# pl0q1n/RustyHGI

Measured on AMD Instinct MI355X. Metric: Mpixels/s encode+decode, 4K grayscale level=4 Medium, higher is better.
Workload: dtype u8

## Files before the change

rustyhgi_amd/csrc/hgi_capi.hip:

```cpp
#include <hip/hip_runtime.h>
#include <stdarg.h>
#include <stdio.h>
#include <stdlib.h>
#include <string.h>
#include <cstring>
#include <thread>
#include <vector>

#include "hgi_framelist.h"
#include "hgi_host.h"
#include "hgi_pitched.h"

using namespace hgi;
using namespace hgi::host;

namespace {
thread_local char g_err[512] = "";
}

namespace hgi {
namespace host {

hgi_status fail(hgi_status st, const char *fmt, ...)
{
    va_list ap;
    va_start(ap, fmt);
    vsnprintf(g_err, sizeof(g_err), fmt, ap);
    va_end(ap);
    return st;
}

}
}

namespace {

#ifndef HGI_ENC_L1_TILE_ROWS
#define HGI_ENC_L1_TILE_ROWS 16
#endif
#ifndef HGI_TILE16_MAX
#define HGI_TILE16_MAX 600
#endif
constexpr uint32_t kConeMinLevels = 6;

}

namespace hgi {
namespace host {

hgi_status ws_ensure(hgi_ctx *c, size_t bytes)
{
    if (bytes <= c->ws_bytes) return HGI_OK;
    HIP_TRY(hipStreamSynchronize(c->stream));
    if (c->ws) HIP_TRY(hipFree(c->ws));
    c->ws = nullptr;
    c->ws_bytes = 0;
    HIP_TRY(hipMalloc(reinterpret_cast<void **>(&c->ws), bytes));
    c->ws_bytes = bytes;
    return HGI_OK;
}

uint8_t *ws_take(hgi_ctx *c, size_t bytes)
{
    size_t off = align_up(c->ws_used, 256);
    if (off + bytes > c->ws_bytes) return nullptr;
    c->ws_used = off + bytes;
    return c->ws + off;
}

struct SubGeom {
    uint32_t sw, sh;
    uint64_t stride;
};

SubGeom sub_geom(uint32_t w, uint32_t h, uint32_t k)
{
    SubGeom g;
    g.sw = (uint32_t)((((uint64_t)w - 1) >> k) + 1);
    g.sh = (uint32_t)((((uint64_t)h - 1) >> k) + 1);
    g.stride = align_up((size_t)g.sw * g.sh, 256);
    return g;
}

struct Split {
    uint32_t k, up, shift;
};

Split split_pyramid(uint32_t levels)
{
    if (levels < kConeMinLevels) return {levels, 0u, 0u};
    if (levels <= 8u) return {4u, levels - 4u, 0u};
    return {4u, 4u, 8u};
}

size_t plane_bytes(const SubGeom &g, size_t batch) { return align_up(batch * g.stride, 256) + 256; }

size_t ws_need_decode(uint32_t w, uint32_t h, uint32_t levels, size_t batch)
{
    const Split sp = split_pyramid(levels);
    if (!sp.shift) return 0;
    const SubGeom g = sub_geom(w, h, sp.shift);
    return 2 * plane_bytes(g, batch) + ws_need_decode(g.sw, g.sh, levels - sp.shift, batch);
}

size_t ws_need_encode(uint32_t w, uint32_t h, uint32_t levels, size_t batch)
{
    const Split sp = split_pyramid(levels);
    if (!sp.shift) return 0;
    const SubGeom g = sub_geom(w, h, sp.shift);
    return 3 * plane_bytes(g, batch) + ws_need_encode(g.sw, g.sh, levels - sp.shift, batch) + ws_need_decode(g.sw, g.sh, levels - sp.shift, batch);
}

size_t ws_need(const hgi_ctx *c, uint32_t w, uint32_t h, uint32_t levels, size_t batch, size_t stride)
{
    if (levels == 0) return 0;
    if (c->path == HGI_PATH_LEVELWISE) return align_up(batch * stride, 256) + 256;
    const size_t e = ws_need_encode(w, h, levels, batch), d = ws_need_decode(w, h, levels, batch);
    return e > d ? e : d;
}

uint32_t use_tile_rows(uint32_t w, uint32_t h, uint32_t k, size_t batch, bool encode, bool plain)
{
    const int forced = HGI_KNOB(HGI_TILE_H, 0);
    const uint64_t tiny_max = (uint64_t)HGI_KNOB(HGI_TILE16_MAX, HGI_TILE16_MAX);
    if (k > (uint32_t)kFusedMaxLevelsSmall) return 64;
    const bool fits16 = k <= (uint32_t)kFusedMaxLevelsTiny;
    if (forced == 16 && fits16) return 16;
    if (forced == 32 || (forced == 16 && !fits16)) return 32;
    if (forced == 64) return 64;
    const uint64_t tx = (w + kTileW - 1) / kTileW;
    const uint64_t tiles64 = tx * ((h + 63) / 64) * batch, tiles32 = tx * ((h + 31) / 32) * batch;
    if (encode && fits16 && tiles32 <= tiny_max) return 16;
    if (tiles64 < 1536) return 32;
    if (encode && plain && k == 1 && w <= 8192) return HGI_ENC_L1_TILE_ROWS;
    const uint64_t interior64 = (uint64_t)(w / kTileW) * (h / 64) * batch * kTileW * 64;
    if (encode && plain && w <= 8192 && interior64 < ((uint64_t)kEncodeEighthsFromGiB << 30)) return 32;
    return 64;
}

bool use_lattice_kernel(const SubGeom &g, size_t batch)
{
    return !HGI_SWITCH(HGI_NO_LATTICE_KERNEL) && lattice_pyramid_fits(g.sw, g.sh, batch);
}

hipError_t launch_encode_fused(const uint8_t *img, uint8_t *grid, const Frames &f, uint32_t k, int interp,
                               const Lut256 &lut, bool ident, const Seeds *seeds, hipStream_t s, uint32_t row_limit = 0)
{
    const uint32_t rows = row_limit && row_limit < f.height ? row_limit : f.height;
    switch (use_tile_rows(f.width, rows, k, f.batch, true, seeds == nullptr)) {
    case 16: return launch_encode_fused_16(img, grid, f, k, interp, lut, ident, seeds, s, row_limit);
    case 32: return launch_encode_fused_32(img, grid, f, k, interp, lut, ident, seeds, s, row_limit);
    default: return launch_encode_fused_64(img, grid, f, k, interp, lut, ident, seeds, s, row_limit);
    }
}

hipError_t launch_decode_fused(const uint8_t *grid, uint8_t *img, const Frames &f, uint32_t k, int interp,
                               const Seeds *seeds, hipStream_t s, uint32_t row_limit = 0, int resident_tiles = -1)
{
    const uint32_t rows = row_limit && row_limit < f.height ? row_limit : f.height;
    switch (use_tile_rows(f.width, rows, k, f.batch, false, seeds == nullptr)) {
    case 16: return launch_decode_fused_16(grid, img, f, k, interp, seeds, s, row_limit, resident_tiles);
    case 32: return launch_decode_fused_32(grid, img, f, k, interp, seeds, s, row_limit, resident_tiles);
    default: return launch_decode_fused_64(grid, img, f, k, interp, seeds, s, row_limit, resident_tiles);
    }
}

Lut256 pack_lut(const uint8_t lut[256])
{
    Lut256 l;
    memcpy(l.w, lut, 256);
    return l;
}

bool is_identity(const uint8_t lut[256])
{
    for (int i = 0; i < 256; ++i)
        if (lut[i] != i) return false;
    return true;
}

hgi_status encode_impl(hgi_ctx *c, const uint8_t *img, uint32_t w, uint32_t h, uint32_t levels, int interp,
                       const uint8_t lut[256], uint8_t *grid, size_t batch, size_t stride)
{
    Frames f = {w, h, (uint64_t)stride, (uint32_t)batch};
    if (levels == 0) {
        for (size_t b = 0; b < batch; ++b)
            HIP_TRY(launch_copy(img + b * stride, grid + b * stride, (size_t)w * h, c->stream));
        return HGI_OK;
    }
    Lut256 l = pack_lut(lut);
    if (c->path == HGI_PATH_LEVELWISE) {
        uint8_t *rec = ws_take(c, batch * stride);
        if (!rec) return fail(HGI_ENOMEM, "scratch exhausted (level-wise reconstruction plane)");
        HIP_TRY(launch_copy(img, rec, (batch - 1) * stride + (size_t)w * h, c->stream));
        HIP_TRY(launch_seed(img, grid, f, levels, c->stream));
        for (uint32_t level = 0; level < levels; ++level)
            HIP_TRY(launch_encode_level(rec, grid, f, levels - level - 1, interp, l, c->stream));
        return HGI_OK;
    }
    const Split sp = split_pyramid(levels);
    if (sp.shift) {
        const SubGeom g = sub_geom(w, h, sp.shift);
        uint8_t *sub_img = ws_take(c, batch * g.stride);
        uint8_t *sub_grid = ws_take(c, batch * g.stride);
        uint8_t *sub_rec = ws_take(c, batch * g.stride);
        if (!sub_img || !sub_grid || !sub_rec) return fail(HGI_ENOMEM, "scratch exhausted (lattice planes)");
        if (use_lattice_kernel(g, batch)) {
            HIP_TRY(launch_lattice_pyramid(img, f, sp.shift, levels - sp.shift, interp, l, is_identity(lut), true, sub_grid, sub_rec,
                                           g.sw, g.sh, g.stride, c->stream));
        } else {
            HIP_TRY(launch_gather_lattice(img, f, sp.shift, sub_img, g.sw, g.sh, g.stride, c->stream));
            HGI_TRY(encode_impl(c, sub_img, g.sw, g.sh, levels - sp.shift, interp, lut, sub_grid, batch, g.stride));
            HGI_TRY(decode_impl(c, sub_grid, g.sw, g.sh, levels - sp.shift, interp, sub_rec, batch, g.stride));
// ... 1124 lines not shown
```

rustyhgi_amd/csrc/hgi_fused_impl.h:

```cpp
#include "hgi_dev.h"
#include "hgi_fastdiv.h"
#include "hgi_knobs.h"
#include "hgi_tilewalk.h"

namespace hgi {
namespace {

using namespace dev;

#ifndef HGI_TILE_H
#define HGI_TILE_H 64
#endif
#define HGI_LOG2(v) ((v) == 32 ? 5 : (v) == 16 ? 4 : (v) == 8 ? 3 : (v) == 4 ? 2 : 1)
#define HGI_CAT2(a, b) a##_##b
#define HGI_CAT(a, b) HGI_CAT2(a, b)
#define HGI_TILED(name) HGI_CAT(name, HGI_TILE_H)
#define HGI_LANE ((int)threadIdx.x)
constexpr int TW = kTileW;
constexpr int TH = HGI_TILE_H;
constexpr int MAXK = TH == 64 ? kFusedMaxLevels : TH == 32 ? kFusedMaxLevelsSmall : kFusedMaxLevelsTiny;
constexpr int NL = kThreads;
constexpr int CH = TW / 16;
constexpr int LCH = 3;
constexpr int HR = 6;
#ifndef HGI_S_PAD
#define HGI_S_PAD 16
#endif
#ifndef HGI_S2_PAD
#define HGI_S2_PAD 8
#endif
constexpr int S = TW + HGI_S_PAD;
constexpr int HP = 40;
constexpr int HCOL = -(HR * HP);
constexpr int S2 = TW / 2 + HGI_S2_PAD;
constexpr int HP2 = 40;
constexpr int RCOL = -(HR * HP2);

__host__ __device__ constexpr int buf_bytes(int nh) { return HR * HP + (TH / 2 + nh) * S; }
__host__ __device__ constexpr int rbuf_bytes(int nh) { return HR * HP2 + (TH / 2 + nh) * S2; }

static_assert(NL == 64 && CH == (1 << LCH) && (TH & (TH - 1)) == 0 && (TH == 64 || TH == 32 || TH == 16) && (1 << MAXK) <= TH, "tile geometry");
static_assert(S % 16 == 0 && (HR * HP) % 16 == 0 && S2 % 8 == 0 && (HR * HP2) % 16 == 0 && HP >= TH / 2 + HR &&
                  HP2 >= TH / 2 + HR && buf_bytes(1) % 16 == 0 && rbuf_bytes(1) % 8 == 0,
              "LDS pitches keep vector alignment");
#ifdef HGI_FUSED_DECODE
static_assert(TH != 64 || 24 * buf_bytes(4) <= 160 * 1024, "LDS budget: 24 decode waves per CU at k = 4");
#endif
#ifdef HGI_FUSED_ENCODE
static_assert(TH != 64 || 18 * (buf_bytes(4) + rbuf_bytes(4) + 256) <= 160 * 1024, "LDS budget: 18 encode waves per CU at k = 4");
#endif

#ifndef HGI_LOAD_AUX
#define HGI_LOAD_AUX 0
#endif
#ifndef HGI_ODD_LOAD_AUX
#define HGI_ODD_LOAD_AUX 2
#endif
#ifndef HGI_STORE_AUX
#define HGI_STORE_AUX 2
#endif
#ifndef HGI_ODD_LATE
#define HGI_ODD_LATE 1
#endif
#ifndef HGI_DEC_CONE_FIRST
#define HGI_DEC_CONE_FIRST 0
#endif
#ifndef HGI_DEC_SHALLOW_WAVES
#define HGI_DEC_SHALLOW_WAVES 20
#endif
#ifndef HGI_DEC_DEEP_WAVES
#define HGI_DEC_DEEP_WAVES 16
#endif
#ifndef HGI_DEC_STREAM_WAVES
#define HGI_DEC_STREAM_WAVES 10
#endif
#ifndef HGI_DEC_STREAM_WAVES_WIDE
#define HGI_DEC_STREAM_WAVES_WIDE 12
#endif
#ifndef HGI_DEC_STREAM_WAVES_L1
#define HGI_DEC_STREAM_WAVES_L1 8
#endif
#ifndef HGI_XCD_MODE
#define HGI_XCD_MODE -1
#endif
#ifndef HGI_XCD_EIGHTHS_FROM_GIB
#define HGI_XCD_EIGHTHS_FROM_GIB kEncodeEighthsFromGiB
#endif
#ifndef HGI_DEC_REVERSE_DEFAULT
#define HGI_DEC_REVERSE_DEFAULT 0
#endif
#ifndef HGI_TILE_BAND
#define HGI_TILE_BAND 8
#endif
#ifndef HGI_HALO_FIRST
#define HGI_HALO_FIRST 0
#endif
#ifndef HGI_HALO_ALL_ROWS
#define HGI_HALO_ALL_ROWS 0
#endif
#ifdef HGI_ANALYZE_K
#define HGI_MARK(name) asm volatile("; HGI_MARK " name)
#else
#define HGI_MARK(name)
#endif
typedef u32 v4u __attribute__((ext_vector_type(4)));
typedef u32 v2u __attribute__((ext_vector_type(2)));
typedef u32 v3u __attribute__((ext_vector_type(3)));

#define HGI_ADDB(dst, K, src, J)                                                                    \
    asm("v_add_u16_sdwa %0, %0, %1 dst_sel:BYTE_" #K " dst_unused:UNUSED_PRESERVE src0_sel:BYTE_" #K \
        " src1_sel:BYTE_" #J                                                                        \
        : "+v"(dst)                                                                                 \
        : "v"(src))

typedef unsigned long long lanemask;
typedef __attribute__((address_space(3))) const u8 lds_cu8;
__device__ __forceinline__ u32 lut_at(u32 d) { return *(lds_cu8 *)(size_t)d; }
#define Q_SUB(d, a, K, p, J)                                                                                   \
    asm("v_sub_u16_sdwa %0, %1, %2 dst_sel:BYTE_0 dst_unused:UNUSED_PAD src0_sel:BYTE_" #K " src1_sel:BYTE_" #J \
        : "=v"(d) : "v"(a), "v"(p))
#define Q_LT(m, a, K, p, J) \
    asm("v_cmp_lt_u16_sdwa %0, %1, %2 src0_sel:BYTE_" #K " src1_sel:BYTE_" #J : "=s"(m) : "v"(a), "v"(p))
#define Q_GT(m, q, np, J) \
    asm("v_cmp_gt_u16_sdwa %0, %1, %2 src0_sel:BYTE_0 src1_sel:BYTE_" #J : "=s"(m) : "v"(q), "v"(np))
#define Q_SEL(out, K, mb, mc, q, d)                                                                    \
    asm("s_xor_b64 vcc, %1, %2\n\tv_cndmask_b32_sdwa %0, %3, %4, vcc dst_sel:BYTE_" #K                 \
        " dst_unused:UNUSED_PRESERVE src0_sel:BYTE_0 src1_sel:BYTE_0"                                  \
        : "+v"(out) : "s"(mb), "s"(mc), "v"(q), "v"(d) : "vcc", "scc")
#define Q_PIX4(slut, P, NP, O0, K0, J0, O1, K1, J1, O2, K2, J2, O3, K3, J3)                              \
    do {                                                                                               \
        u32 d0_, d1_, d2_, d3_;                                                                        \
        lanemask b0_, b1_, b2_, b3_, c0_, c1_, c2_, c3_;                                               \
        Q_SUB(d0_, O0, K0, P, J0); Q_SUB(d1_, O1, K1, P, J1); Q_SUB(d2_, O2, K2, P, J2); Q_SUB(d3_, O3, K3, P, J3); \
        u32 q0_ = lut_at(d0_), q1_ = lut_at(d1_), q2_ = lut_at(d2_), q3_ = lut_at(d3_);                \
        Q_LT(b0_, O0, K0, P, J0); Q_LT(b1_, O1, K1, P, J1); Q_LT(b2_, O2, K2, P, J2); Q_LT(b3_, O3, K3, P, J3); \
        Q_GT(c0_, q0_, NP, J0); Q_GT(c1_, q1_, NP, J1); Q_GT(c2_, q2_, NP, J2); Q_GT(c3_, q3_, NP, J3); \
        Q_SEL(O0, K0, b0_, c0_, q0_, d0_); Q_SEL(O1, K1, b1_, c1_, q1_, d1_);                          \
        Q_SEL(O2, K2, b2_, c2_, q2_, d2_); Q_SEL(O3, K3, b3_, c3_, q3_, d3_);                          \
    } while (0)
// ... 856 lines not shown
}

__device__ __forceinline__ u8 *uniform_ptr(const u8 *p)
{
    const u64 a = reinterpret_cast<u64>(p);
    const u32 lo = __builtin_amdgcn_readfirstlane((u32)a), hi = __builtin_amdgcn_readfirstlane((u32)(a >> 32));
    return reinterpret_cast<u8 *>(((u64)hi << 32) | lo);
}

__device__ __forceinline__ Buf make_buf(const u8 *fr, u8 *out, u32 W, u32 H, Tile tl, u32 tail)
{
    Buf b;
    const u32 bytes = W * H;
    b.rs = __builtin_amdgcn_make_buffer_rsrc(uniform_ptr(fr), 0, bytes + tail, 0x00020000);
    b.rd = __builtin_amdgcn_make_buffer_rsrc(uniform_ptr(out), 0, bytes, 0x00020000);
    b.W = W;
    b.base = __builtin_amdgcn_readfirstlane(tl.Y0 * W + tl.X0);
    return b;
}

__device__ __forceinline__ Tile fast_tile(u32 t, const TileGrid &g)
{
    t = __builtin_amdgcn_readfirstlane(walk_position(t, g));
    const WalkTile w = walk_fast_tile(t, g);
    Tile tl;
    tl.frame = w.frame;
    tl.X0 = w.tx * TW;
    tl.Y0 = w.ty * TH;
    return tl;
}

__device__ __forceinline__ Tile edge_tile(u32 e, const TileGrid &g)
{
    const WalkTile w = walk_edge_tile(e, g);
    Tile tl;
    tl.frame = w.frame;
    tl.X0 = w.tx * TW;
    tl.Y0 = w.ty * TH;
    return tl;
}

struct TileCtx {
    Tile tl;
    Buf b;
};

#ifndef HGI_ARGS_EARLY
#define HGI_ARGS_EARLY 1
#endif
__device__ __forceinline__ void args_early(const u8 *src, const u8 *dst, const Frames &f, const TileGrid &g, u32 aligned, u32 k)
{
#if HGI_ARGS_EARLY
    asm volatile("" ::"s"(k), "s"(g.full_x), "s"(g.full_y), "s"(g.tiles_x), "s"(g.tiles_y));
    asm volatile("" ::"s"(src), "s"(dst), "s"(f.width), "s"(f.height), "s"(f.frame_stride), "s"(aligned), "s"(g.nedge), "s"(g.nf), "s"(g.xmode),
                 "s"(g.rr_own), "s"(g.rr_tail0), "s"(g.P), "s"(g.fd_P.m), "s"(g.fd_P.s1), "s"(g.fd_P.s2), "s"(g.reverse), "s"(g.tpf), "s"(g.fd_tpf.m),
                 "s"(g.fd_tpf.s1), "s"(g.fd_tpf.s2), "s"(g.nfull), "s"(g.rem_rows), "s"(g.band), "s"(g.ex), "s"(g.fd_band.m), "s"(g.fd_band.s1),
                 "s"(g.fd_band.s2), "s"(g.fd_rem.m), "s"(g.fd_rem.s1), "s"(g.fd_rem.s2));
#endif
}

__device__ __forceinline__ TileCtx fast_ctx(u32 t, const u8 *src, u8 *dst, const Frames &f, const TileGrid &g, u32 tail)
{
    TileCtx c;
    c.tl = fast_tile(t, g);
    c.b = make_buf(src + (size_t)c.tl.frame * f.frame_stride, dst + (size_t)c.tl.frame * f.frame_stride, f.width,
                   f.height, c.tl, tail);
    return c;
}

struct SeedRegs {
    u32 rec, q;
    int bx, by;
    bool on;
};

template <bool WANT_Q>
__device__ __forceinline__ SeedRegs seed_issue(const Seeds &sd, Tile tl, u32 k)
{
    const int ext = k >= 2 ? 2 : 1;
    const int nbx = (TW >> k) + ext, nby = (TH >> k) + ext;
    const int i = HGI_LANE;
    SeedRegs r;
    r.by = i / nbx;
    r.bx = i - r.by * nbx;
    r.on = i < nbx * nby;
    r.rec = r.q = 0;
    const u32 sx = (tl.X0 >> k) + r.bx, sy = (tl.Y0 >> k) + r.by;
    if (r.on && sx < sd.sw && sy < sd.sh) {
        const size_t at = (size_t)tl.frame * sd.stride + (size_t)sy * sd.sw + sx;
        r.rec = sd.rec[at];
        if (WANT_Q) r.q = sd.q[at];
    }
    return r;
}

__device__ __forceinline__ void dec_seed_commit(u8 *buf, const SeedRegs &r, u32 k)
{
    if (r.on) buf[laddr(r.bx << k, r.by << k)] = (u8)r.rec;
    LDS_ORDER();
}

constexpr int kConeMaxUp = 4;
__host__ __device__ constexpr int cone_n(int tile_px, int t)
{
    const int c = tile_px >> 4;
    int n = c + 2;
    for (int i = 0; i < t; ++i) n = (c % (2 << i) == 0 ? (n - 1) / 2 : n / 2) + 2;
// ... 386 lines not shown
        if (tl.X0 + TW <= W && !(H & 1u))
            enc_tile_edge<INTERP, IDENT, 1>(buf, rbuf, slut, cur, st.o, k, W, H);
        else
            enc_tile_edge<INTERP, IDENT, 2>(buf, rbuf, slut, cur, st.o, k, W, H);
        return;
    }
    if (!IDENT) reinterpret_cast<u32 *>(slut)[HGI_LANE] = lut.w[HGI_LANE];
    stage_tile_generic(buf, fr, W, H, tl, nh, (aligned & 1u) != 0);
    LDS_ORDER();
    lattice_from_buf(buf, rbuf, nh);
    LDS_ORDER();
    if (SEEDED == 2) seeds = cone_finish<INTERP, true, IDENT>(cone, buf, rbuf, sd.up, slut);
    enc_seed_commit<SEEDED>(buf, rbuf, seeds, k);
    for (int s = 1 << (k - 1); s >= 2; s >>= 1) {
        enc_cells<INTERP, IDENT, true>(buf, rbuf, slut, s, tl, W, H);
        enc_halo_pass<INTERP, IDENT>(buf, rbuf, slut, s, tl, W, H);
        LDS_ORDER();
    }
    enc_fine_generic<INTERP, IDENT>(buf, rbuf, slut, fr, out, tl, W, H, (aligned & 1u) != 0);
}

inline bool ptr16(const void *p) { return (reinterpret_cast<uintptr_t>(p) & 15u) == 0; }

struct FusedGeom {
    TileGrid g;
    u32 aligned;
    bool ok;
};

FusedGeom fused_geom(const void *a, const void *b, const Frames &f, u32 row_limit)
{
    FusedGeom r;
    TileGrid &g = r.g;
    g.tiles_x = (f.width + TW - 1) / TW;
    g.tiles_y = (f.height + TH - 1) / TH;
    if (row_limit && row_limit / TH < g.tiles_y) g.tiles_y = row_limit / TH;
    const bool aligned = f.width % 16 == 0 && f.frame_stride % 16 == 0 && ptr16(a) && ptr16(b);
    const bool fits32 = ((u64)f.height + 2 * TH + 64) * f.width + 1024 < (1ull << 32);
    const bool force_checked = HGI_SWITCH(HGI_FORCE_CHECKED);
    const uintptr_t end = reinterpret_cast<uintptr_t>(a) + (uintptr_t)(f.batch - 1) * f.frame_stride + (uintptr_t)f.width * f.height;
    const bool dword_rows = f.width % 4 == 0;
    const bool tail_ok = ((end - 1) >> 12) == ((end + 2) >> 12) && (f.batch == 1 || f.frame_stride >= (u64)f.width * f.height);
    const bool fast = fits32 && (dword_rows || tail_ok) && !force_checked;
    g.full_x = fast ? f.width / TW : 0;
    g.full_y = fast ? f.height / TH : 0;
    if (g.full_y > g.tiles_y) g.full_y = g.tiles_y;
    if (g.full_x == 0 || g.full_y == 0) g.full_x = g.full_y = 0;
    const u64 all = (u64)g.tiles_x * g.tiles_y * f.batch, nfast = (u64)g.full_x * g.full_y * f.batch;
    r.ok = all > 0 && all + 8 < (1ull << 31);
    g.nfast = (u32)nfast;
    g.nedge = (u32)(all - nfast);
    g.reverse = 0;
    g.band = HGI_TILE_BAND;
    g.xmode = 0;
    r.aligned = (aligned ? 1u : 0u) | (fast ? 2u : 0u) | (fast && !dword_rows ? 4u : 0u);
#ifdef HGI_TIMELINE
    g.timeline = g_timeline;
#endif
    return r;
}

inline u32 band_rows(const Frames &f, bool encode)
{
    const int forced = encode ? HGI_KNOB(HGI_ENC_BAND, 0) : HGI_KNOB(HGI_DEC_BAND, 0);
    if (forced > 0) return (u32)forced;
    const u64 cap = encode ? (4u << 20) : (2u << 20);
    u32 rows = HGI_TILE_BAND;
    while (rows > 1 && (u64)rows * TH * f.width > cap) rows >>= 1;
    return rows;
}


inline size_t lds_for_waves(size_t lds, int waves)
{
    if (waves <= 0) return lds;
    const size_t cap = ((size_t)160 * 1024 / (size_t)waves) & ~(size_t)255;
    return cap > lds ? cap : lds;
}

inline u32 xcd_mode(const TileGrid &g, bool encode)
{
    const int forced = HGI_KNOB(HGI_XCD_MODE, HGI_XCD_MODE);
    if (forced >= 0) return (u32)forced;
    return encode && (u64)g.nfast * TW * TH >= ((u64)HGI_XCD_EIGHTHS_FROM_GIB << 30) ? 0u : 1u;
}

}

#ifndef HGI_FUSED_NO_LAUNCHERS
#ifdef HGI_FUSED_DECODE
hipError_t HGI_TILED(launch_decode_fused)(const uint8_t *grid, uint8_t *img, const Frames &f, uint32_t k, int interp,
                                          const Seeds *seeds, hipStream_t s, uint32_t row_limit, int resident_tiles)
{
    FusedGeom r = fused_geom(grid, img, f, row_limit);
    if (!r.ok || k < 1 || k > (u32)MAXK) return hipErrorInvalidValue;
    r.g.reverse = HGI_KNOB(HGI_DEC_REVERSE, HGI_DEC_REVERSE_DEFAULT) ? 1u : 0u;
    r.g.band = band_rows(f, false);
    r.g.xmode = xcd_mode(r.g, false);
    finish_grid(r.g);
    const TileGrid &g = r.g;
    if (seeds && k < (uint32_t)kSeededMinLevels) return hipErrorInvalidValue;
    Seeds sd = seeds ? *seeds : Seeds{nullptr, nullptr, 0, 0, 0, 0};
    const bool cone = seeds && seeds->up != 0;
    if (cone && (k != 4 || sd.up > (u32)kConeMaxUp)) return hipErrorInvalidValue;
    if (seeds && !cone && !seeds->rec) return hipErrorInvalidValue;
    const dim3 b(NL);
    const int nh = k >= 2 ? (int)k : 1;
    const int dec_waves_forced = HGI_KNOB(HGI_DEC_WAVES, -1);
    const u64 tiles = (u64)g.nfast + g.nedge;
    int dec_waves = 0;
    if (resident_tiles >= 0)
        dec_waves = resident_tiles;
    else if (dec_waves_forced >= 0)
        dec_waves = dec_waves_forced;
    else if (tiles < 8192)
        dec_waves = 0;
    else if (!seeds)
        dec_waves = f.width > 4096 || k > 4 ? HGI_DEC_STREAM_WAVES_WIDE : k == 1 ? HGI_DEC_STREAM_WAVES_L1 : HGI_DEC_STREAM_WAVES;
    else
        dec_waves = tiles >= 65536 ? HGI_DEC_DEEP_WAVES : HGI_DEC_SHALLOW_WAVES;
    const size_t lds = lds_for_waves((size_t)buf_bytes(nh), dec_waves);
    const dim3 blocks(((g.nedge + 7u) & ~7u) + g.nfast);
#define HGI_DEC(I, SE) hipLaunchKernelGGL((k_dec_tiles<I, SE, TH>), blocks, b, lds, s, grid, img, f, k, sd, g, r.aligned)
#define HGI_DEC_I(I)                                                     \
    do {                                                                 \
        if (!seeds) HGI_DEC(I, 0);                                       \
        else if (cone) HGI_DEC(I, 2);                                    \
        else if constexpr (TH == 64) HGI_DEC(I, 1);                      \
        else return hipErrorInvalidValue;                                \
    } while (0)
    if (interp == kInterpCrossed) HGI_DEC_I(kInterpCrossed); else HGI_DEC_I(kInterpLeftTop);
#undef HGI_DEC_I
#undef HGI_DEC
    return hipGetLastError();
}

#endif

#ifdef HGI_FUSED_ENCODE
namespace {
hipError_t static_lds_is_empty(const void *kernel)
{
    hipFuncAttributes a;
    const hipError_t e = hipFuncGetAttributes(&a, kernel);
    if (e != hipSuccess) return e;
    return a.sharedSizeBytes == 0 ? hipSuccess : hipErrorInvalidDeviceFunction;
}
}

hipError_t HGI_TILED(launch_encode_fused)(const uint8_t *img, uint8_t *grid, const Frames &f, uint32_t k, int interp,
                                          const Lut256 &lut, bool ident, const Seeds *seeds, hipStream_t s, uint32_t row_limit)
{
    FusedGeom r = fused_geom(img, grid, f, row_limit);
    if (!r.ok || k < 1 || k > (u32)MAXK) return hipErrorInvalidValue;
    r.g.band = band_rows(f, true);
    r.g.xmode = xcd_mode(r.g, true);
    finish_grid(r.g);
    const TileGrid &g = r.g;
    if (seeds && k < (uint32_t)kSeededMinLevels) return hipErrorInvalidValue;
    Seeds sd = seeds ? *seeds : Seeds{nullptr, nullptr, 0, 0, 0, 0};
    const bool cone = seeds && seeds->up != 0;
    if (cone && (k != 4 || sd.up > (u32)kConeMaxUp)) return hipErrorInvalidValue;
    if (seeds && (!seeds->rec != !seeds->q || (!cone && !seeds->rec))) return hipErrorInvalidValue;
    const dim3 b(NL);
    const int nh = k >= 2 ? (int)k : 1;
    const int enc_waves = HGI_KNOB(HGI_ENC_WAVES, 0);
    const size_t lds = lds_for_waves((size_t)buf_bytes(nh) + ((rbuf_bytes(nh) + 15) & ~15) + 256, enc_waves);
    const dim3 blocks(((g.nedge + 7u) & ~7u) + g.nfast);
#define HGI_ENC(I, ID, SE)                                                                                        \
    do {                                                                                                          \
        static const hipError_t lds0 = static_lds_is_empty(reinterpret_cast<const void *>(&k_enc_tiles<I, ID, SE, TH>)); \
        if (lds0 != hipSuccess) return lds0;                                                                      \
        hipLaunchKernelGGL((k_enc_tiles<I, ID, SE, TH>), blocks, b, lds, s, img, grid, f, k, lut, sd, g, r.aligned); \
    } while (0)
#define HGI_ENC_ID(I, ID)                                                     \
    do {                                                                      \
        if (cone) HGI_ENC(I, ID, 2);                                          \
        else if (!seeds) HGI_ENC(I, ID, 0);                                   \
        else if constexpr (TH == 64) HGI_ENC(I, ID, 1);                       \
        else return hipErrorInvalidValue;                                     \
    } while (0)
#define HGI_ENC_I(I)                                                          \
    do {                                                                      \
        if (ident) HGI_ENC_ID(I, true); else HGI_ENC_ID(I, false);            \
    } while (0)
    if (interp == kInterpCrossed) HGI_ENC_I(kInterpCrossed); else HGI_ENC_I(kInterpLeftTop);
#undef HGI_ENC_I
#undef HGI_ENC_ID
#undef HGI_ENC
    return hipGetLastError();
}

#endif
#endif

}
```

rustyhgi_amd/csrc/hgi_kernels.h:

```cpp
#pragma once
#include <hip/hip_runtime.h>
#include <stddef.h>
#include <stdint.h>

#include "hgi_huffman_host.h"

namespace hgi {

constexpr int kInterpLeftTop = 0;
constexpr int kInterpCrossed = 1;

constexpr int kTileW = 128;
constexpr int kFusedMaxLevels = 6;
constexpr int kFusedMaxLevelsSmall = 5;
constexpr int kFusedMaxLevelsTiny = 4;
constexpr int kSeededMinLevels = 4;
constexpr int kThreads = 64;
constexpr int kEncodeEighthsFromGiB = 4;

struct Lut256 {
    uint32_t w[64];
};

struct Frames {
    uint32_t width, height;
    uint64_t frame_stride;
    uint32_t batch;
};

struct Seeds {
    const uint8_t *rec;
    const uint8_t *q;
    uint32_t sw, sh;
    uint64_t stride;
    uint32_t up;
};

#ifdef HGI_TIMELINE
extern uint64_t *g_timeline;
#endif

hipError_t launch_seed(const uint8_t *src, uint8_t *dst, const Frames &f, uint32_t levels,
                       hipStream_t s);
hipError_t launch_decode_level(const uint8_t *grid, uint8_t *img, const Frames &f, uint32_t log2sub,
                               int interp, hipStream_t s);
hipError_t launch_encode_level(uint8_t *rec, uint8_t *grid, const Frames &f, uint32_t log2sub,
                               int interp, const Lut256 &lut, hipStream_t s);

#define HGI_DECLARE_FUSED(TH)                                                                                      \
    hipError_t launch_decode_fused_##TH(const uint8_t *grid, uint8_t *img, const Frames &f, uint32_t k, int interp, \
                                        const Seeds *seeds, hipStream_t s, uint32_t row_limit, int resident_tiles); \
    hipError_t launch_encode_fused_##TH(const uint8_t *img, uint8_t *grid, const Frames &f, uint32_t k, int interp, \
                                        const Lut256 &lut, bool lut_is_identity, const Seeds *seeds, hipStream_t s, \
                                        uint32_t row_limit);
HGI_DECLARE_FUSED(64)
HGI_DECLARE_FUSED(32)
HGI_DECLARE_FUSED(16)
#undef HGI_DECLARE_FUSED

struct RegionRect {
    uint32_t x0, y0, width, height;
    uint64_t out_pitch, out_frame_stride;
};
hipError_t launch_decode_region(const uint8_t *grid, uint8_t *out, const Frames &f, const RegionRect &r, uint32_t k, int interp,
                                const Seeds *seeds, hipStream_t s);

struct ScaledView {
    uint32_t width, height, shift;
    uint64_t row_pitch, frame_bytes, frame_stride;
    uint32_t batch;
    uint64_t out_pitch, out_frame_stride;
// ... 40 lines not shown
```

rustyhgi_amd/csrc/hgi_planes.hip:

```cpp
#include <hip/hip_runtime.h>
#include <stdarg.h>
#include <stdio.h>
#include <stdlib.h>
#include <array>
#include <mutex>
#include <utility>
#include <vector>

#include "hgi_host.h"
#include "hgi_lineup.h"

using namespace hgi;
using namespace hgi::host;
using hgi::lineup::arrange;

namespace {

hgi_status probe_pair_ms(hgi_ctx *c, const uint8_t *prev, uint8_t *cand, size_t bytes, float *ms)
{
    const uint32_t w = 4096;
    size_t rows = bytes / w;
    if (rows > (2u << 20) / 4) rows = (2u << 20) / 4;
    rows &= ~(size_t)63;
    const uint32_t h = (uint32_t)rows;
    constexpr int kWarm = 2, kTimed = 4;
    struct Occupancy {
        hgi_ctx *c;
        explicit Occupancy(hgi_ctx *ctx) : c(ctx) { c->probe_resident_tiles = 0; }
        ~Occupancy() { c->probe_resident_tiles = -1; }
    } occupancy(c);
    for (int i = 0; i < kWarm + kTimed; ++i) {
        if (i == kWarm) HIP_TRY(hipEventRecord(c->ev_probe[0], c->stream));
        c->ws_used = 0;
        HGI_TRY(decode_impl(c, prev, w, h, 4, HGI_INTERP_LEFTTOP, cand, 1, (size_t)w * h));
    }
    HIP_TRY(hipEventRecord(c->ev_probe[1], c->stream));
    HIP_TRY(hipEventSynchronize(c->ev_probe[1]));
    HIP_TRY(hipEventElapsedTime(ms, c->ev_probe[0], c->ev_probe[1]));
    *ms /= kTimed;
    return HGI_OK;
}

constexpr size_t kGiB = (size_t)1 << 30;
constexpr float kFastRatio = 0.972f, kUnsureLo = 0.962f, kUnsureHi = 0.985f;
constexpr int kMaxCandidates = 10;
constexpr size_t kComposeAbove = kGiB;
constexpr size_t kChunk = kGiB;

struct Yardstick {
    void *ref = nullptr;
    uint8_t *lo = nullptr, *hi = nullptr;
    size_t span = 0;

    hgi_status make(size_t span_bytes)
    {
        span = span_bytes;
        size_t ref_bytes = 1;
        while (ref_bytes < 2 * span) ref_bytes <<= 1;
        if (hipMalloc(&ref, ref_bytes) != hipSuccess) {
            (void)hipGetLastError();
            ref = nullptr;
            return HGI_ENOMEM;
        }
// ... 454 lines not shown
                        if (trace) fprintf(stderr, "hgi_planes_alloc: offset %zu, plane %u: chunk %d exchanged for %zu\n", m, i + 1, rows[m][i + 1], u);
                        used[(size_t)rows[m][i + 1]] = 0;
                        used[u] = 1;
                        rows[m][i + 1] = (int)u;
                        yes = true;
                    }
                }
                ok = yes;
            }
    }
    for (uint32_t i = 0; i < count; ++i) {
        Composed p;
        p.va = nullptr;
        p.bytes = n * kChunk;
        p.device = c->device;
        void *va = nullptr;
        PL_TRY(hipMemAddressReserve(&va, p.bytes, 0, nullptr, 0));
        p.va = va;
        made.push_back(p);
        for (size_t m = 0; m < n; ++m) {
            const size_t j = (size_t)rows[m][i];
            if (mapped[j]) {
                hipError_t e = hipMemUnmap(stage + j * kChunk, kChunk);
                if (e != hipSuccess) return bail(fail(HGI_EDEVICE, "hipMemUnmap: %s", hipGetErrorString(e)));
                mapped[j] = 0;
            }
            hipError_t e = hipMemMap(static_cast<uint8_t *>(va) + m * kChunk, kChunk, 0, h[j], 0);
            if (e != hipSuccess) return bail(fail(HGI_EDEVICE, "hipMemMap: %s", hipGetErrorString(e)));
            made.back().chunks.push_back(h[j]);
            owned[j] = 1;
        }
        hipError_t e = hipMemSetAccess(va, p.bytes, &acc, 1);
        if (e != hipSuccess) return bail(fail(HGI_EDEVICE, "hipMemSetAccess: %s", hipGetErrorString(e)));
    }
#undef PL_TRY
    for (size_t j = 0; j < h.size(); ++j)
        if (!owned[j]) {
            if (mapped[j]) (void)hipMemUnmap(stage + j * kChunk, kChunk);
            mapped[j] = 0;
            (void)hipMemRelease(h[j]);
        }
    cleanup(true);
    {
        std::lock_guard<std::mutex> lock(g_mu);
        for (uint32_t i = 0; i < count; ++i) {
            planes[i] = made[i].va;
            g_composed.push_back(made[i]);
        }
    }
    if (separated) *separated = ok ? 1 : 0;
    return HGI_OK;
}

}

extern "C" {

hgi_status hgi_probe_pair_u8_dev(hgi_ctx *c, const void *d_src, void *d_dst, size_t bytes, float *ms)
{
    if (!c || !d_src || !d_dst || !ms) return fail(HGI_EINVAL, "NULL argument");
    if (bytes < 4096 * 64) return fail(HGI_EINVAL, "probe needs at least 256 KiB");
    const uintptr_t a = reinterpret_cast<uintptr_t>(d_src), b = reinterpret_cast<uintptr_t>(d_dst);
    if (a < b + bytes && b < a + bytes) return fail(HGI_EINVAL, "probe buffers overlap");
    HIP_TRY(hipSetDevice(c->device));
    HGI_TRY(ws_ensure(c, ws_need(c, 4096, 4096, 4, 1, (size_t)4096 * 4096)));
    return probe_pair_ms(c, static_cast<const uint8_t *>(d_src), static_cast<uint8_t *>(d_dst), bytes, ms);
}

hgi_status hgi_planes_alloc(hgi_ctx *c, size_t bytes, uint32_t count, void **planes, int *separated)
{
    if (!c || !planes) return fail(HGI_EINVAL, "NULL argument");
    if (separated) *separated = 0;
    for (uint32_t i = 0; i < count; ++i) planes[i] = nullptr;
    if (count == 0 || bytes == 0) return HGI_OK;
    HIP_TRY(hipSetDevice(c->device));
    const bool placing = count > 1 && !getenv("HGI_NO_PLACEMENT");
    c->planes_report[0] = 0;
    if (!placing || bytes < ((size_t)128 << 20)) {
        snprintf(c->planes_report, sizeof c->planes_report, "plain allocations (%s)", placing ? "planes below 128 MiB are not probed" : count > 1 ? "HGI_NO_PLACEMENT" : "one plane");
        return alloc_plain(bytes, count, planes);
    }
    if (bytes > kComposeAbove) return alloc_composed(c, bytes, count, planes, separated);
    if (bytes < kGiB) {
        const hgi_status st = alloc_whole(c, kGiB, count, planes, separated);
        if (st != HGI_ENOMEM) return st;
        if (separated) *separated = 0;
        snprintf(c->planes_report, sizeof c->planes_report, "plain allocations (no room for candidates of 1 GiB)");
        return alloc_plain(bytes, count, planes);
    }
    return alloc_whole(c, bytes, count, planes, separated);
}

const char *hgi_planes_report(hgi_ctx *c) { return c ? c->planes_report : ""; }

hgi_status hgi_planes_free(hgi_ctx *c, uint32_t count, void **planes)
{
    if (!c || (!planes && count)) return fail(HGI_EINVAL, "NULL argument");
    HIP_TRY(hipSetDevice(c->device));
    for (uint32_t i = 0; i < count; ++i) {
        if (!planes[i]) continue;
        Composed mine;
        mine.va = nullptr;
        {
            std::lock_guard<std::mutex> lock(g_mu);
            for (size_t k = 0; k < g_composed.size(); ++k)
                if (g_composed[k].va == planes[i]) {
                    mine = g_composed[k];
                    g_composed.erase(g_composed.begin() + (long)k);
                    break;
                }
        }
        if (mine.va) {
            HIP_TRY(hipDeviceSynchronize());
            release_composed(mine);
        } else {
            HIP_TRY(hipFree(planes[i]));
        }
        planes[i] = nullptr;
    }
    return HGI_OK;
}

}
```

rustyhgi_amd/csrc/hgi_tilewalk.h:

```cpp
#pragma once
#include <stdint.h>

#include "hgi_fastdiv.h"

#if defined(__HIPCC__)
#define HGI_WALK_FN __host__ __device__ __forceinline__
#else
#define HGI_WALK_FN inline
#endif
#ifndef HGI_TILE_ORDER
#define HGI_TILE_ORDER 0
#endif

namespace hgi {
namespace {

struct TileGrid {
    uint32_t tiles_x, tiles_y;
    uint32_t full_x, full_y;
    uint32_t nfast, nedge;
    uint32_t reverse;
    uint32_t band;
    uint32_t xmode;
    uint32_t ex, nf;
    uint32_t tpf, P, nfull, rem_rows;
    uint32_t rr_own, rr_tail0;
    FastDiv fd_tpf, fd_P, fd_band, fd_rem, fd_ex;
#ifdef HGI_TIMELINE
    uint64_t *timeline;
#endif
};

struct WalkTile {
    uint32_t frame, tx, ty;
};

HGI_WALK_FN uint32_t range_first(uint32_t ntiles, uint32_t x) { return x * (ntiles >> 3) + (x < (ntiles & 7u) ? x : (ntiles & 7u)); }

HGI_WALK_FN uint32_t walk_position(uint32_t t, const TileGrid &g) { return g.reverse ? g.nf - 1u - t : t; }

HGI_WALK_FN WalkTile walk_fast_tile(uint32_t t, const TileGrid &g)
{
    WalkTile tl;
    tl.frame = fdiv(t, g.fd_tpf);
    const uint32_t tt = t - tl.frame * g.tpf;
    uint32_t ty, tx;
#if HGI_TILE_ORDER == 0
    ty = fdiv(tt, g.fd_ex);
    tx = tt - ty * g.ex;
#else
    {
        uint32_t rows, row0, r;
        if (tt < g.nfull) {
            const uint32_t band = fdiv(tt, g.fd_P);
            r = tt - band * g.P;
            row0 = band * g.band;
            rows = g.band;
            tx = fdiv(r, g.fd_band);
        } else {
            rows = g.rem_rows;
            r = tt - g.nfull;
            row0 = g.full_y - rows;
            tx = fdiv(r, g.fd_rem);
        }
        ty = row0 + (r - tx * rows);
    }
#endif
    tl.tx = tx;
    tl.ty = ty;
    return tl;
}

HGI_WALK_FN WalkTile walk_edge_tile(uint32_t e, const TileGrid &g)
{
    const uint32_t right = (g.tiles_x - g.full_x) * g.tiles_y;
    const uint32_t epf = right + g.full_x * (g.tiles_y - g.full_y);
    WalkTile tl;
    tl.frame = e / epf;
    uint32_t i = e - tl.frame * epf, tx, ty;
    if (i < right) {
        const uint32_t w = g.tiles_x - g.full_x;
        ty = i / w;
        tx = g.full_x + (i - ty * w);
    } else {
        i -= right;
        ty = g.full_y + i / g.full_x;
        tx = i % g.full_x;
    }
    tl.tx = tx;
    tl.ty = ty;
    return tl;
}

struct BlockRole {
    bool edge, idle;
    uint32_t index;
};

HGI_WALK_FN BlockRole walk_block_role(uint32_t b, const TileGrid &g)
{
    const uint32_t ne8 = (g.nedge + 7u) & ~7u;
    BlockRole r;
    r.edge = b < ne8;
    r.idle = r.edge && b >= g.nedge;
    const uint32_t fb = b - ne8;
    r.index = r.edge ? b : range_first(g.nf, fb & 7u) + (fb >> 3);
    if (!r.edge && g.xmode == 1) {
        const uint32_t x = fb & 7u, sq = fb >> 3;
        if (sq < g.rr_own) {
            const uint32_t round = fdiv(sq, g.fd_P);
            r.index = (round * 8u + x) * g.P + (sq - round * g.P);
        } else {
            r.index = g.rr_tail0 + range_first(g.nf - g.rr_tail0, x) + (sq - g.rr_own);
        }
    }
    return r;
}

inline void finish_grid(TileGrid &g)
{
    g.ex = g.full_x;
    g.nf = g.nfast;
    if (g.band < 1) g.band = 1;
    g.tpf = g.ex * g.full_y;
    g.P = g.band * g.ex;
    g.nfull = (g.full_y / g.band) * g.P;
    g.rem_rows = g.full_y % g.band;
    g.fd_tpf = make_fastdiv(g.tpf);
    g.fd_P = make_fastdiv(g.P);
    g.fd_band = make_fastdiv(g.band);
    g.fd_rem = make_fastdiv(g.rem_rows);
    g.fd_ex = make_fastdiv(g.ex);
    g.rr_own = g.rr_tail0 = 0;
    if (g.xmode != 1 || g.rem_rows != 0 || g.P == 0 || g.nf == 0) {
        g.xmode = 0;
    } else {
        const uint32_t nb8 = (g.nf / g.P) & ~7u;
        g.rr_own = (nb8 >> 3) * g.P;
        g.rr_tail0 = nb8 * g.P;
    }
}

}
}
```

Measured before the change: 1.603 million.

## Pick tile rows and XCD front count from buffer placement-aware launch policy

Adds a registry of plane allocations so launches can tell whether src and dst are separately placed planes from one allocation call. A new launch policy uses this placement plus interior size to choose tile rows and a number of XCD 'fronts' (1, 2, 4 or 8), and the tile-to-block mapping gains a grouped-front variant. The aim is to fit the XCD work distribution to how memory is placed. The cost is a mutex-guarded lookup on every launch, and decode now always gets 64-row tiles with one front.

```diff
diff --git a/rustyhgi_amd/csrc/hgi_capi.hip b/rustyhgi_amd/csrc/hgi_capi.hip
--- a/rustyhgi_amd/csrc/hgi_capi.hip
+++ b/rustyhgi_amd/csrc/hgi_capi.hip
@@ -9,6 +9,7 @@
 
 #include "hgi_framelist.h"
 #include "hgi_host.h"
+#include "hgi_placement.h"
 #include "hgi_pitched.h"
 
 using namespace hgi;
@@ -35,9 +36,6 @@
 
 namespace {
 
-#ifndef HGI_ENC_L1_TILE_ROWS
-#define HGI_ENC_L1_TILE_ROWS 16
-#endif
 #ifndef HGI_TILE16_MAX
 #define HGI_TILE16_MAX 600
 #endif
@@ -119,7 +117,8 @@
     return e > d ? e : d;
 }
 
-uint32_t use_tile_rows(uint32_t w, uint32_t h, uint32_t k, size_t batch, bool encode, bool plain)
+uint32_t use_tile_rows(uint32_t w, uint32_t h, uint32_t k, size_t batch, bool encode, bool plain, const void *src, const void *dst,
+                       uint64_t frame_stride)
 {
     const int forced = HGI_KNOB(HGI_TILE_H, 0);
     const uint64_t tiny_max = (uint64_t)HGI_KNOB(HGI_TILE16_MAX, HGI_TILE16_MAX);
@@ -132,10 +131,11 @@
     const uint64_t tiles64 = tx * ((h + 63) / 64) * batch, tiles32 = tx * ((h + 31) / 32) * batch;
     if (encode && fits16 && tiles32 <= tiny_max) return 16;
     if (tiles64 < 1536) return 32;
-    if (encode && plain && k == 1 && w <= 8192) return HGI_ENC_L1_TILE_ROWS;
-    const uint64_t interior64 = (uint64_t)(w / kTileW) * (h / 64) * batch * kTileW * 64;
-    if (encode && plain && w <= 8192 && interior64 < ((uint64_t)kEncodeEighthsFromGiB << 30)) return 32;
-    return 64;
+    const uint64_t interior64 = interior_tile_bytes(w, h, batch);
+    const int forced_placed = HGI_KNOB(HGI_PLACED, -1);
+    const bool placed = forced_placed >= 0 ? forced_placed != 0
+                                           : batch > 0 && placement::placed(src, dst, (batch - 1) * (size_t)frame_stride + (size_t)w * h);
+    return launch_policy(encode, plain, interior64, w, k, placed).tile_rows;
 }
 
 bool use_lattice_kernel(const SubGeom &g, size_t batch)
@@ -147,7 +147,7 @@
                                const Lut256 &lut, bool ident, const Seeds *seeds, hipStream_t s, uint32_t row_limit = 0)
 {
     const uint32_t rows = row_limit && row_limit < f.height ? row_limit : f.height;
-    switch (use_tile_rows(f.width, rows, k, f.batch, true, seeds == nullptr)) {
+    switch (use_tile_rows(f.width, rows, k, f.batch, true, seeds == nullptr, img, grid, f.frame_stride)) {
     case 16: return launch_encode_fused_16(img, grid, f, k, interp, lut, ident, seeds, s, row_limit);
     case 32: return launch_encode_fused_32(img, grid, f, k, interp, lut, ident, seeds, s, row_limit);
     default: return launch_encode_fused_64(img, grid, f, k, interp, lut, ident, seeds, s, row_limit);
@@ -158,7 +158,7 @@
                                const Seeds *seeds, hipStream_t s, uint32_t row_limit = 0, int resident_tiles = -1)
 {
     const uint32_t rows = row_limit && row_limit < f.height ? row_limit : f.height;
-    switch (use_tile_rows(f.width, rows, k, f.batch, false, seeds == nullptr)) {
+    switch (use_tile_rows(f.width, rows, k, f.batch, false, seeds == nullptr, grid, img, f.frame_stride)) {
     case 16: return launch_decode_fused_16(grid, img, f, k, interp, seeds, s, row_limit, resident_tiles);
     case 32: return launch_decode_fused_32(grid, img, f, k, interp, seeds, s, row_limit, resident_tiles);
     default: return launch_decode_fused_64(grid, img, f, k, interp, seeds, s, row_limit, resident_tiles);
diff --git a/rustyhgi_amd/csrc/hgi_fused_impl.h b/rustyhgi_amd/csrc/hgi_fused_impl.h
--- a/rustyhgi_amd/csrc/hgi_fused_impl.h
+++ b/rustyhgi_amd/csrc/hgi_fused_impl.h
@@ -1,6 +1,9 @@
+#include <stdio.h>
+
 #include "hgi_dev.h"
 #include "hgi_fastdiv.h"
 #include "hgi_knobs.h"
+#include "hgi_placement.h"
 #include "hgi_tilewalk.h"
 
 namespace hgi {
@@ -83,8 +86,8 @@
 #ifndef HGI_XCD_MODE
 #define HGI_XCD_MODE -1
 #endif
-#ifndef HGI_XCD_EIGHTHS_FROM_GIB
-#define HGI_XCD_EIGHTHS_FROM_GIB kEncodeEighthsFromGiB
+#ifndef HGI_XCD_FRONTS
+#define HGI_XCD_FRONTS 0
 #endif
 #ifndef HGI_DEC_REVERSE_DEFAULT
 #define HGI_DEC_REVERSE_DEFAULT 0
@@ -1047,7 +1050,7 @@
 {
 #if HGI_ARGS_EARLY
     asm volatile("" ::"s"(k), "s"(g.full_x), "s"(g.full_y), "s"(g.tiles_x), "s"(g.tiles_y));
-    asm volatile("" ::"s"(src), "s"(dst), "s"(f.width), "s"(f.height), "s"(f.frame_stride), "s"(aligned), "s"(g.nedge), "s"(g.nf), "s"(g.xmode),
+    asm volatile("" ::"s"(src), "s"(dst), "s"(f.width), "s"(f.height), "s"(f.frame_stride), "s"(aligned), "s"(g.nedge), "s"(g.nf), "s"(g.xmode), "s"(g.fronts),
                  "s"(g.rr_own), "s"(g.rr_tail0), "s"(g.P), "s"(g.fd_P.m), "s"(g.fd_P.s1), "s"(g.fd_P.s2), "s"(g.reverse), "s"(g.tpf), "s"(g.fd_tpf.m),
                  "s"(g.fd_tpf.s1), "s"(g.fd_tpf.s2), "s"(g.nfull), "s"(g.rem_rows), "s"(g.band), "s"(g.ex), "s"(g.fd_band.m), "s"(g.fd_band.s1),
                  "s"(g.fd_band.s2), "s"(g.fd_rem.m), "s"(g.fd_rem.s1), "s"(g.fd_rem.s2));
@@ -1540,6 +1543,7 @@
     g.nedge = (u32)(all - nfast);
     g.reverse = 0;
     g.band = HGI_TILE_BAND;
+    g.fronts = 8;
     g.xmode = 0;
     r.aligned = (aligned ? 1u : 0u) | (fast ? 2u : 0u) | (fast && !dword_rows ? 4u : 0u);
 #ifdef HGI_TIMELINE
@@ -1566,11 +1570,25 @@
     return cap > lds ? cap : lds;
 }
 
-inline u32 xcd_mode(const TileGrid &g, bool encode)
-{
-    const int forced = HGI_KNOB(HGI_XCD_MODE, HGI_XCD_MODE);
-    if (forced >= 0) return (u32)forced;
-    return encode && (u64)g.nfast * TW * TH >= ((u64)HGI_XCD_EIGHTHS_FROM_GIB << 30) ? 0u : 1u;
+inline bool launch_is_placed(const void *src, const void *dst, const Frames &f)
+{
+    const int forced = HGI_KNOB(HGI_PLACED, -1);
+    if (forced >= 0) return forced != 0;
+    return placement::placed(src, dst, (size_t)(f.batch - 1) * f.frame_stride + (size_t)f.width * f.height);
+}
+
+inline u32 xcd_fronts(const Frames &f, u32 row_limit, u32 k, bool encode, bool plain, const void *src, const void *dst)
+{
+    const bool placed = launch_is_placed(src, dst, f);
+    const u32 rows = row_limit && row_limit < f.height ? row_limit : f.height;
+    u32 fronts = launch_policy(encode, plain, interior_tile_bytes(f.width, rows, f.batch), f.width, k, placed).fronts;
+    const int mode = HGI_KNOB(HGI_XCD_MODE, HGI_XCD_MODE), forced = HGI_KNOB(HGI_XCD_FRONTS, HGI_XCD_FRONTS);
+    if (mode >= 0) fronts = mode == 1 ? 1u : 8u;
+    if (forced == 1 || forced == 2 || forced == 4 || forced == 8) fronts = (u32)forced;
+    if (HGI_SWITCH(HGI_POLICY_REPORT))
+        fprintf(stderr, "hgi policy: %s %u x %u x %u levels %u placed %d tile rows %d fronts %u\n", encode ? "encode" : "decode", f.batch, f.width,
+                f.height, k, placed ? 1 : 0, TH, fronts);
+    return fronts;
 }
 
 }
@@ -1584,7 +1602,7 @@
     if (!r.ok || k < 1 || k > (u32)MAXK) return hipErrorInvalidValue;
     r.g.reverse = HGI_KNOB(HGI_DEC_REVERSE, HGI_DEC_REVERSE_DEFAULT) ? 1u : 0u;
     r.g.band = band_rows(f, false);
-    r.g.xmode = xcd_mode(r.g, false);
+    r.g.fronts = xcd_fronts(f, row_limit, k, false, seeds == nullptr, grid, img);
     finish_grid(r.g);
     const TileGrid &g = r.g;
     if (seeds && k < (uint32_t)kSeededMinLevels) return hipErrorInvalidValue;
@@ -1642,7 +1660,7 @@
     FusedGeom r = fused_geom(img, grid, f, row_limit);
     if (!r.ok || k < 1 || k > (u32)MAXK) return hipErrorInvalidValue;
     r.g.band = band_rows(f, true);
-    r.g.xmode = xcd_mode(r.g, true);
+    r.g.fronts = xcd_fronts(f, row_limit, k, true, seeds == nullptr, img, grid);
     finish_grid(r.g);
     const TileGrid &g = r.g;
     if (seeds && k < (uint32_t)kSeededMinLevels) return hipErrorInvalidValue;
diff --git a/rustyhgi_amd/csrc/hgi_kernels.h b/rustyhgi_amd/csrc/hgi_kernels.h
--- a/rustyhgi_amd/csrc/hgi_kernels.h
+++ b/rustyhgi_amd/csrc/hgi_kernels.h
@@ -4,6 +4,7 @@
 #include <stdint.h>
 
 #include "hgi_huffman_host.h"
+#include "hgi_policy.h"
 
 namespace hgi {
 
@@ -16,7 +17,6 @@
 constexpr int kFusedMaxLevelsTiny = 4;
 constexpr int kSeededMinLevels = 4;
 constexpr int kThreads = 64;
-constexpr int kEncodeEighthsFromGiB = 4;
 
 struct Lut256 {
     uint32_t w[64];
diff --git a/rustyhgi_amd/csrc/hgi_placement.h b/rustyhgi_amd/csrc/hgi_placement.h
--- /dev/null
+++ b/rustyhgi_amd/csrc/hgi_placement.h
@@ -0,0 +1,60 @@
+#pragma once
+#include <stddef.h>
+#include <stdint.h>
+
+#include <mutex>
+#include <vector>
+
+namespace hgi {
+namespace placement {
+
+struct Plane {
+    uintptr_t base;
+    size_t bytes;
+    uint64_t call;
+    uint32_t index;
+    bool separated;
+};
+
+inline std::mutex g_mu;
+inline std::vector<Plane> g_planes;
+inline uint64_t g_calls = 0;
+
+inline void add_call(void *const *planes, uint32_t count, size_t bytes, bool separated)
+{
+    std::lock_guard<std::mutex> lock(g_mu);
+    const uint64_t call = ++g_calls;
+    for (uint32_t i = 0; i < count; ++i)
+        if (planes[i]) g_planes.push_back(Plane{reinterpret_cast<uintptr_t>(planes[i]), bytes, call, i, separated});
+}
+
+inline void remove(const void *plane)
+{
+    std::lock_guard<std::mutex> lock(g_mu);
+    const uintptr_t p = reinterpret_cast<uintptr_t>(plane);
+    for (size_t k = 0; k < g_planes.size(); ++k)
+        if (g_planes[k].base == p) {
+            g_planes.erase(g_planes.begin() + (long)k);
+            return;
+        }
+}
+
+inline const Plane *find_locked(uintptr_t p, size_t bytes)
+{
+    for (const Plane &pl : g_planes)
+        if (p >= pl.base && bytes <= pl.bytes && p - pl.base <= pl.bytes - bytes) return &pl;
+    return nullptr;
+}
+
+inline bool placed(const void *src, const void *dst, size_t bytes)
+{
+    std::lock_guard<std::mutex> lock(g_mu);
+    if (g_planes.empty()) return false;
+    const Plane *a = find_locked(reinterpret_cast<uintptr_t>(src), bytes);
+    if (!a || !a->separated) return false;
+    const Plane *b = find_locked(reinterpret_cast<uintptr_t>(dst), bytes);
+    return b && b->call == a->call && (b->index == a->index + 1u || a->index == b->index + 1u);
+}
+
+}
+}
diff --git a/rustyhgi_amd/csrc/hgi_planes.hip b/rustyhgi_amd/csrc/hgi_planes.hip
--- a/rustyhgi_amd/csrc/hgi_planes.hip
+++ b/rustyhgi_amd/csrc/hgi_planes.hip
@@ -9,6 +9,7 @@
 
 #include "hgi_host.h"
 #include "hgi_lineup.h"
+#include "hgi_placement.h"
 
 using namespace hgi;
 using namespace hgi::host;
@@ -569,25 +570,8 @@
     return HGI_OK;
 }
 
-}
-
-extern "C" {
-
-hgi_status hgi_probe_pair_u8_dev(hgi_ctx *c, const void *d_src, void *d_dst, size_t bytes, float *ms)
-{
-    if (!c || !d_src || !d_dst || !ms) return fail(HGI_EINVAL, "NULL argument");
-    if (bytes < 4096 * 64) return fail(HGI_EINVAL, "probe needs at least 256 KiB");
-    const uintptr_t a = reinterpret_cast<uintptr_t>(d_src), b = reinterpret_cast<uintptr_t>(d_dst);
-    if (a < b + bytes && b < a + bytes) return fail(HGI_EINVAL, "probe buffers overlap");
-    HIP_TRY(hipSetDevice(c->device));
-    HGI_TRY(ws_ensure(c, ws_need(c, 4096, 4096, 4, 1, (size_t)4096 * 4096)));
-    return probe_pair_ms(c, static_cast<const uint8_t *>(d_src), static_cast<uint8_t *>(d_dst), bytes, ms);
-}
-
-hgi_status hgi_planes_alloc(hgi_ctx *c, size_t bytes, uint32_t count, void **planes, int *separated)
-{
-    if (!c || !planes) return fail(HGI_EINVAL, "NULL argument");
-    if (separated) *separated = 0;
+hgi_status planes_alloc(hgi_ctx *c, size_t bytes, uint32_t count, void **planes, int *separated)
+{
     for (uint32_t i = 0; i < count; ++i) planes[i] = nullptr;
     if (count == 0 || bytes == 0) return HGI_OK;
     HIP_TRY(hipSetDevice(c->device));
@@ -608,6 +592,33 @@
     return alloc_whole(c, bytes, count, planes, separated);
 }
 
+}
+
+extern "C" {
+
+hgi_status hgi_probe_pair_u8_dev(hgi_ctx *c, const void *d_src, void *d_dst, size_t bytes, float *ms)
+{
+    if (!c || !d_src || !d_dst || !ms) return fail(HGI_EINVAL, "NULL argument");
+    if (bytes < 4096 * 64) return fail(HGI_EINVAL, "probe needs at least 256 KiB");
+    const uintptr_t a = reinterpret_cast<uintptr_t>(d_src), b = reinterpret_cast<uintptr_t>(d_dst);
+    if (a < b + bytes && b < a + bytes) return fail(HGI_EINVAL, "probe buffers overlap");
+    HIP_TRY(hipSetDevice(c->device));
+    HGI_TRY(ws_ensure(c, ws_need(c, 4096, 4096, 4, 1, (size_t)4096 * 4096)));
+    return probe_pair_ms(c, static_cast<const uint8_t *>(d_src), static_cast<uint8_t *>(d_dst), bytes, ms);
+}
+
+hgi_status hgi_planes_alloc(hgi_ctx *c, size_t bytes, uint32_t count, void **planes, int *separated)
+{
+    if (!c || !planes) return fail(HGI_EINVAL, "NULL argument");
+    int sep = 0;
+    if (separated) *separated = 0;
+    const hgi_status st = planes_alloc(c, bytes, count, planes, &sep);
+    if (st != HGI_OK) return st;
+    if (separated) *separated = sep;
+    placement::add_call(planes, count, bytes, sep != 0 || HGI_SWITCH(HGI_TEST_PLACED_PLAIN));
+    return HGI_OK;
+}
+
 const char *hgi_planes_report(hgi_ctx *c) { return c ? c->planes_report : ""; }
 
 hgi_status hgi_planes_free(hgi_ctx *c, uint32_t count, void **planes)
@@ -616,6 +627,7 @@
     HIP_TRY(hipSetDevice(c->device));
     for (uint32_t i = 0; i < count; ++i) {
         if (!planes[i]) continue;
+        placement::remove(planes[i]);
         Composed mine;
         mine.va = nullptr;
         {
diff --git a/rustyhgi_amd/csrc/hgi_policy.h b/rustyhgi_amd/csrc/hgi_policy.h
--- /dev/null
+++ b/rustyhgi_amd/csrc/hgi_policy.h
@@ -0,0 +1,34 @@
+#pragma once
+#include <stdint.h>
+
+namespace hgi {
+
+constexpr int kEncodeEighthsFromGiB = 4;
+constexpr int kUnplacedEighthsAboveGiB = 8;
+
+#ifndef HGI_ENC_L1_TILE_ROWS
+#define HGI_ENC_L1_TILE_ROWS 16
+#endif
+
+inline uint64_t interior_tile_bytes(uint32_t width, uint32_t rows, uint64_t batch) { return (uint64_t)(width / 128u) * (rows / 64u) * batch * 128u * 64u; }
+
+struct LaunchPolicy {
+    uint32_t tile_rows;
+    uint32_t fronts;
+};
+
+inline LaunchPolicy launch_policy(bool encode, bool plain, uint64_t interior_bytes, uint32_t width, uint32_t levels, bool placed)
+{
+    LaunchPolicy p = {64u, 1u};
+    if (!encode) return p;
+    const bool unplaced_rule = !placed && plain && width <= 8192;
+    const bool big = unplaced_rule ? interior_bytes > ((uint64_t)kUnplacedEighthsAboveGiB << 30) : interior_bytes >= ((uint64_t)kEncodeEighthsFromGiB << 30);
+    p.fronts = big ? 8u : 1u;
+    if (plain && width <= 8192) {
+        if (levels == 1) p.tile_rows = HGI_ENC_L1_TILE_ROWS;
+        else if (!big) p.tile_rows = 32u;
+    }
+    return p;
+}
+
+}
diff --git a/rustyhgi_amd/csrc/hgi_tilewalk.h b/rustyhgi_amd/csrc/hgi_tilewalk.h
--- a/rustyhgi_amd/csrc/hgi_tilewalk.h
+++ b/rustyhgi_amd/csrc/hgi_tilewalk.h
@@ -21,10 +21,12 @@
     uint32_t nfast, nedge;
     uint32_t reverse;
     uint32_t band;
+    uint32_t fronts;
     uint32_t xmode;
     uint32_t ex, nf;
     uint32_t tpf, P, nfull, rem_rows;
     uint32_t rr_own, rr_tail0;
+    uint32_t lg_group;
     FastDiv fd_tpf, fd_P, fd_band, fd_rem, fd_ex;
 #ifdef HGI_TIMELINE
     uint64_t *timeline;
@@ -107,11 +109,26 @@
     r.index = r.edge ? b : range_first(g.nf, fb & 7u) + (fb >> 3);
     if (!r.edge && g.xmode == 1) {
         const uint32_t x = fb & 7u, sq = fb >> 3;
-        if (sq < g.rr_own) {
-            const uint32_t round = fdiv(sq, g.fd_P);
-            r.index = (round * 8u + x) * g.P + (sq - round * g.P);
+        if (g.fronts == 1) {
+            if (sq < g.rr_own) {
+                const uint32_t round = fdiv(sq, g.fd_P);
+                r.index = (round * 8u + x) * g.P + (sq - round * g.P);
+            } else {
+                r.index = g.rr_tail0 + range_first(g.nf - g.rr_tail0, x) + (sq - g.rr_own);
+            }
         } else {
-            r.index = g.rr_tail0 + range_first(g.nf - g.rr_tail0, x) + (sq - g.rr_own);
+            const uint32_t lg = g.lg_group, j = x & ((1u << lg) - 1u), x0 = x - j;
+            const uint32_t s0 = range_first(g.nf, x0), s1 = range_first(g.nf, x0 + (1u << lg));
+            uint32_t a = (fdiv(s0 + g.P - 1u, g.fd_P)) * g.P;
+            if (a > s1) a = s1;
+            const uint32_t own = (fdiv(s1 - a, g.fd_P) >> lg) * g.P;
+            if (sq < own) {
+                const uint32_t round = fdiv(sq, g.fd_P);
+                r.index = a + ((round << lg) + j) * g.P + (sq - round * g.P);
+            } else {
+                const uint32_t p = range_first(g.nf, x) - s0 - j * own + (sq - own), head = a - s0;
+                r.index = p < head ? s0 + p : a + (own << lg) + (p - head);
+            }
         }
     }
     return r;
@@ -131,13 +148,19 @@
     g.fd_band = make_fastdiv(g.band);
     g.fd_rem = make_fastdiv(g.rem_rows);
     g.fd_ex = make_fastdiv(g.ex);
-    g.rr_own = g.rr_tail0 = 0;
-    if (g.xmode != 1 || g.rem_rows != 0 || g.P == 0 || g.nf == 0) {
+    g.rr_own = g.rr_tail0 = g.lg_group = 0;
+    if (g.fronts == 0) g.fronts = g.xmode == 1 ? 1u : 8u;
+    if ((g.fronts != 1 && g.fronts != 2 && g.fronts != 4) || g.rem_rows != 0 || g.P == 0 || g.nf == 0) {
+        g.fronts = 8;
         g.xmode = 0;
-    } else {
+    } else if (g.fronts == 1) {
+        g.xmode = 1;
         const uint32_t nb8 = (g.nf / g.P) & ~7u;
         g.rr_own = (nb8 >> 3) * g.P;
         g.rr_tail0 = nb8 * g.P;
+    } else {
+        g.xmode = 1;
+        g.lg_group = g.fronts == 2 ? 2u : 1u;
     }
 }
 
```

New measurement: 1.602 million. Within noise of the previous version (-0.1%).
